# AIM-Harvard/pyradiomics

Hardware: AMD Instinct MI355X
Metric: Mvoxels/s for GLCM+GLRLM build, 512^3 vol @32 bins (higher is better)
Workload: dtype u8 levels / u32 counts / f64 out; 1 GPU; GLCM+GLRLM matrix build, 512^3 int32+uint8 volume resident in HBM, 32 grey levels, full mask, 13 angles, uniform levels; one volume per GPU (batch sharding, no collective); size=512, levels=32, dist=uniform, deferred_mode=pipeline

## Files before the change

pyradiomics_amd/csrc/kernels_sweep.h:

```cpp
#pragma once
#include "prad_runtime.h"

namespace prad {

typedef unsigned int u32;
typedef unsigned long long u64;

__global__ void __launch_bounds__(256) pack_levels_kernel(const int *__restrict__ image,
                                                          const uint8_t *__restrict__ mask, long long n, int NX,
                                                          int pitch, int padw, int Ng,
                                                          uint8_t *__restrict__ levels, int *__restrict__ flags,
                                                          int vec_ok, int shift, uint8_t *__restrict__ rowzero = nullptr) {
  const long long tid = (long long)blockIdx.x * blockDim.x + threadIdx.x;
  const long long nthreads = (long long)gridDim.x * blockDim.x;
  const bool linear = (padw == 0 && pitch == NX);
  int bad = 0;
  long long done = 0;
  if (vec_ok) {
    const long long n16 = n >> 4;
    const int upr = NX >> 4;
    const int4 *im4 = reinterpret_cast<const int4 *>(image);
    const uint4 *mk4 = reinterpret_cast<const uint4 *>(mask);
    for (long long t = tid; t < n16; t += nthreads) {
      const uint4 m = mk4[t];
// ... 66 lines not shown
  long long sM, sU;
  int LXc;
  long long chunks;
};
#define PRAD_MAX_SWEEP 16
struct SweepSet {
  int count;
  SweepDesc d[PRAD_MAX_SWEEP];
};

#define PRAD_LONG_BINS 64
struct HistLayout {
  int Ng, RS;
  bool fused;
  int glrlm0;
  int g0, RL;
  int dummy0;
  int words;
};
__host__ __device__ inline HistLayout hist_layout(bool glcm, bool glrlm, bool fused, int Ng, int RS) {
  HistLayout h;
  h.Ng = Ng;
  h.RS = RS;
  h.fused = fused;
  h.g0 = 0;
  h.RL = 0;
  if (fused) {
    h.glrlm0 = 0;
    h.g0 = (Ng + 1) * (RS + 1) * (Ng + 1);
    h.RL = PRAD_LONG_BINS;
    h.dummy0 = h.g0 + Ng * h.RL;
  } else {
    h.glrlm0 = glcm ? Ng * Ng : 0;
    h.dummy0 = h.glrlm0 + (glrlm ? RS * Ng : 0);
  }
  h.words = h.dummy0 + 64;
  return h;
}

__device__ __forceinline__ int select_i32(bool cond, int a, int b) {
  asm volatile("" : "+v"(a), "+v"(b));
  return cond ? a : b;
}

typedef __attribute__((address_space(3))) u32 lds_u32;
__device__ __forceinline__ void lds_bump(int lds_addr) {
#ifdef PRAD_DBG_NOBUMP
  asm volatile("" ::"v"(lds_addr));
  return;
#endif
  __hip_atomic_fetch_add((lds_u32 *)(size_t)(unsigned)lds_addr, 1u, __ATOMIC_RELAXED, __HIP_MEMORY_SCOPE_WORKGROUP);
}

template <bool DO_GLCM, bool DO_GLRLM, bool LONG, bool FUSED>
struct Walker {
  u32 *rl_long;
  int Ng4, Nr;
  int cG, cR;
  int rl_limit;
  int dummy;
  int prev;
  int prowG;
  int rlN;
  int nmask;

  __device__ __forceinline__ void init(u32 *lds_, const HistLayout &h, int Nr_, u32 *rl_long_, int lane) {
    const int base = (int)(unsigned)(size_t)((lds_u32 *)lds_);
    rl_long = rl_long_;
    Ng4 = 4 * h.Ng;
    Nr = Nr_;
    cG = base - 4 * (h.Ng + 1);
    cR = base + 4 * (h.glrlm0 - (h.Ng + 1));
    rl_limit = h.RS * Ng4 + cR;
    dummy = base + 4 * (h.dummy0 + lane);
  }
  __device__ __forceinline__ void begin_line() {
    prev = 0;
    prowG = cG;
    rlN = Ng4 + cR;
    nmask = 0;
  }
  __device__ __forceinline__ bool risky(int steps) const { return LONG && DO_GLRLM && rlN + steps * Ng4 > rl_limit; }
  template <bool CHECK = true>
  __device__ __forceinline__ void step(int cur) {
    const bool pnz = prev != 0, cnz = cur != 0;
    if (DO_GLCM) {
      lds_bump((pnz && cnz) ? prowG + (cur << 2) : dummy);
      prowG = __mul24(cur, Ng4) + cG;
    }
    if (DO_GLRLM) {
      const bool chg = cur != prev;
      const bool emit = chg && pnz;
      if (LONG && CHECK) {
        const bool lng = rlN > rl_limit;
        lds_bump((emit && !lng) ? rlN + (prev << 2) : dummy);
        if (emit && lng) atomicAdd(&rl_long[(size_t)(prev - 1) * Nr + ((rlN - cR) / Ng4 - 1)], 1u);
      } else {
        lds_bump(emit ? rlN + (prev << 2) : dummy);
      }
      rlN = select_i32(chg, Ng4 + cR, rlN + Ng4);
      nmask += cnz;
    }
    prev = cur;
  }
  __device__ __forceinline__ bool end_line() {
    step<true>(0);
// ... 540 lines not shown
  if ((int)blockIdx.x < nb1) {
    const long long idx = (long long)blockIdx.x * blockDim.x + threadIdx.x;
    const long long total = (long long)Ng * Ng * Na;
    if (idx >= total) return;
    const int a = (int)(idx % Na);
    const long long ij = idx / Na;
    const int i = (int)(ij / Ng), j = (int)(ij - (long long)i * Ng);
    if (i == j) return;
    glcm_out[idx] = (double)glcm_acc[(size_t)a * Ng * Ng + ij];
    return;
  }
  const int pair = ((int)blockIdx.x - nb1) * 4 + (int)(threadIdx.x >> 6), lane = threadIdx.x & 63;
  if (pair >= Ng * Na) return;
  const int i = pair % Ng, a = pair / Ng;
  u32 *row = glrlm_acc + ((size_t)a * Ng + i) * Nr;
  unsigned long long pairs = 0, longer = 0;
  int found = 0;
  for (int r = lane; r < Nr; r += 64) {
    const u32 v = row[r];
    pairs += (unsigned long long)r * v;
    if (r > 0) longer += v;
    found |= (r > 0 && v != 0);
  }
  const u32 *grow = glcm_acc + ((size_t)a * Ng + i) * Ng;
  for (int j = lane; j < Ng; j += 64) found |= (grow[j] != 0);
  for (int o = 32; o > 0; o >>= 1) pairs += __shfl_xor(pairs, o);
  if (lane == 0) glcm_out[((size_t)i * Ng + i) * Na + a] = (double)pairs;
  if (__ballot(found) != 0 && lane == 0) multi[a] = 1;
  if (restore_from >= 0 && a != restore_from) {
    const u32 *xrow = glrlm_acc + ((size_t)restore_from * Ng + i) * Nr;
    unsigned long long nvox = 0;
    for (int r = lane; r < Nr; r += 64) nvox += (unsigned long long)(r + 1) * xrow[r];
    for (int o = 32; o > 0; o >>= 1) {
      nvox += __shfl_xor(nvox, o);
      longer += __shfl_xor(longer, o);
    }
    if (lane == 0) row[0] = (u32)(nvox - (pairs + longer));
  }
}

__global__ void finalize_glrlm_kernel(const u32 *__restrict__ acc, const int *__restrict__ multi, int Ng, int Nr,
                                      int Na, double *__restrict__ out, const int *__restrict__ flags = nullptr,
                                      int *__restrict__ sticky = nullptr) {
  if (sticky && blockIdx.x == 0 && threadIdx.x == 0 && (flags[0] || flags[2])) sticky[0] = 1;
  const long long idx = (long long)blockIdx.x * blockDim.x + threadIdx.x;
  const long long total = (long long)Ng * Nr * Na;
  if (idx >= total) return;
  const int a = (int)(idx % Na);
  const long long gr = idx / Na;
  const int r = (int)(gr % Nr);
  out[idx] = (r == 0 && !multi[a]) ? 0.0 : (double)acc[(size_t)a * Ng * Nr + gr];
}

}
```

pyradiomics_amd/csrc/kernels_sweepfw.h:

```cpp
#pragma once
#include "kernels_sweep.h"

namespace prad {

enum FwPhase { FP_INIT, FP_GRAB, FP_CTRL, FP_ISSUE, FP_WAIT_ROWS, FP_WAIT_PACK, FP_GROUP, FP_PACK, FP_SLOW, FP_FLUSH, FP_DRAIN,
               FP_TOTAL, FP_REALTIME, FP_NGROUP, FP_NGROUP_PACK, FP_NSLOW, FP_COUNT };
#ifdef PRAD_FW_STAMPS
__device__ unsigned long long prad_fw_stamps[2 * 8192 * FP_COUNT];
struct FwClock {
  unsigned long long last, first, rt0;
  unsigned acc[FP_COUNT];
  __device__ __forceinline__ void start() {
#pragma unroll
    for (int i = 0; i < FP_COUNT; i++) acc[i] = 0;
    rt0 = __builtin_amdgcn_s_memrealtime();
    first = last = __builtin_readcyclecounter();
  }
  template <int PH>
  __device__ __forceinline__ void lap() {
    const unsigned long long now = __builtin_readcyclecounter();
    acc[PH] += (unsigned)(now - last);
    last = now;
  }
  template <int PH>
  __device__ __forceinline__ void count() { acc[PH]++; }
  __device__ __forceinline__ void store(int slot) {
    acc[FP_TOTAL] = (unsigned)(__builtin_readcyclecounter() - first);
    acc[FP_REALTIME] = (unsigned)(__builtin_amdgcn_s_memrealtime() - rt0);
    const unsigned w = blockIdx.x * (blockDim.x >> 6) + (threadIdx.x >> 6);
    if ((threadIdx.x & 63) == 0 && w < 8192) {
#pragma unroll
      for (int i = 0; i < FP_COUNT; i++) prad_fw_stamps[((size_t)slot * 8192 + w) * FP_COUNT + i] = acc[i];
    }
  }
};
#else
struct FwClock {
  __device__ __forceinline__ void start() {}
  template <int PH>
  __device__ __forceinline__ void lap() {}
  template <int PH>
  __device__ __forceinline__ void count() {}
  __device__ __forceinline__ void store(int) {}
};
#endif

struct FwDesc {
  int slot;
  int NM, NU;
  int du, dx;
  long long sM, sU;
  int CL, pieces;
  int chunks;
  int dom_kind;
};
struct FwSet {
  int count;
  int NX;
  int pitch;
  int nrows;
  int xcd;
  int first_block[PRAD_MAX_SWEEP + 1];
  FwDesc d[PRAD_MAX_SWEEP];
};

struct PackJob {
  const int *image;
  const uint8_t *mask;
  uint8_t *levels;
  uint8_t *levels16;
  uint8_t *rowzero;
  int *flags;
  long long n16;
  int NX, Ng;
  int every;
};

#define PRAD_FW_U 8
#ifndef PRAD_FW_MAXG
#define PRAD_FW_MAXG 4
#endif
#define PRAD_FW_WORK_STRIDE 64
#define PRAD_FW_DOMAINS 8
__host__ __device__ inline size_t fw_lds_bytes(const HistLayout &h) { return 4 * ((size_t)h.words + (size_t)(h.Ng + 1)); }


struct FwTab {
  u32 *rl_long;
  int Nr, P4, Q, lenlim, gB, RL4, RS, RL, dummy0b, alive0, deadmax;
  unsigned Qinv;
  __device__ __forceinline__ void init(const HistLayout &h, int Nr_, u32 *rl_long_) {
    rl_long = rl_long_;
    Nr = Nr_;
    Q = 4 * (h.Ng + 1);
    P4 = (h.RS + 1) * (h.Ng + 1);
    lenlim = (h.RS + 1) * Q;
// ... 671 lines not shown
          ri -= (long long)du * NU * sUr;
          zpos = 65;
          wrap = false;
          continue;
        }
        t++;
        zpos++;
        row += du;
        off += delta;
        ri += dri;
        if (du != 0 && (row < 0 || row >= NU)) wrap = true;
      }
    }
  }
};

template <bool ZA>
__device__ __forceinline__ void fw_row_word(const FwTab &T, u32 one, int &s, u32 c, u32 x) {
  int t;
#define PRAD_FW_RCOL(J)                                                                                          \
  "v_cmpx_ne_u32_sdwa vcc, %[c], %[x] src0_sel:BYTE_" #J " src1_sel:BYTE_" #J "\n\t"                             \
  "v_add_u32_sdwa %[t], %[s], %[c] dst_sel:DWORD dst_unused:UNUSED_PAD src0_sel:DWORD src1_sel:BYTE_" #J "\n\t"   \
  "v_mul_u32_u24_sdwa %[s], %[P4], %[c] dst_sel:DWORD dst_unused:UNUSED_PAD src0_sel:DWORD src1_sel:BYTE_" #J "\n\t" \
  "v_cmpx_ne_u32_sdwa vcc, %[x], %[z] src0_sel:BYTE_" #J " src1_sel:DWORD\n\t"                                  \
  "ds_add_u32 %[t], %[one]\n\t"                                                                                  \
  "s_mov_b64 exec, -1\n\t"                                                                                       \
  "v_add_u32 %[s], %[Q], %[s]\n\t"
#define PRAD_FW_RCOL_NZ(J)                                                                                       \
  "v_cmpx_ne_u32_sdwa vcc, %[c], %[x] src0_sel:BYTE_" #J " src1_sel:BYTE_" #J "\n\t"                             \
  "v_add_u32_sdwa %[t], %[s], %[c] dst_sel:DWORD dst_unused:UNUSED_PAD src0_sel:DWORD src1_sel:BYTE_" #J "\n\t"   \
  "ds_add_u32 %[t], %[one]\n\t"                                                                                  \
  "v_mul_u32_u24_sdwa %[s], %[P4], %[c] dst_sel:DWORD dst_unused:UNUSED_PAD src0_sel:DWORD src1_sel:BYTE_" #J "\n\t" \
  "s_mov_b64 exec, -1\n\t"                                                                                       \
  "v_add_u32 %[s], %[Q], %[s]\n\t"
  if (ZA) {
    u32 z = 0;
    asm volatile("" : "+v"(z));
    asm volatile(PRAD_FW_RCOL(0) PRAD_FW_RCOL(1) PRAD_FW_RCOL(2) PRAD_FW_RCOL(3)
                 : [s] "+v"(s), [t] "=&v"(t)
                 : [c] "v"(c), [x] "v"(x), [one] "v"(one), [P4] "s"(T.P4), [Q] "s"(T.Q), [z] "v"(z)
                 : "vcc", "memory");
  } else {
    asm volatile(PRAD_FW_RCOL_NZ(0) PRAD_FW_RCOL_NZ(1) PRAD_FW_RCOL_NZ(2) PRAD_FW_RCOL_NZ(3)
                 : [s] "+v"(s), [t] "=&v"(t)
                 : [c] "v"(c), [x] "v"(x), [one] "v"(one), [P4] "s"(T.P4), [Q] "s"(T.Q)
                 : "vcc", "memory");
  }
#undef PRAD_FW_RCOL
#undef PRAD_FW_RCOL_NZ
}

template <bool LONG, bool ZA>
__device__ __forceinline__ void fw_rows_role(const HistLayout &h, const FwTab &T, u32 *lds, const uint8_t *__restrict__ L,
                                             long long nrows, int NX, int pitch, int bx, int nblocks) {
  const int lane = threadIdx.x & 63, wave = threadIdx.x >> 6, wpb = blockDim.x >> 6;
  const int dummy = T.dummy0b + 4 * lane;
  u32 one = 1;
  asm volatile("" : "+v"(one));
  uint8_t *tile = reinterpret_cast<uint8_t *>(lds) + ((fw_lds_bytes(h) + 15) & ~(size_t)15) + (size_t)wave * 64 * PRAD_ROW_PITCH;
  const int RSTEP = nrows >= 4096 ? 8 : 1;
  const long long ngroups = RSTEP == 8 ? ((nrows + 511) / 512) * 8 : (nrows + 63) / 64;
  const long long nwaves = (long long)nblocks * wpb;
  const bool vec16 = (pitch & 15) == 0 && ((uintptr_t)L & 15) == 0;
  for (long long grp = (long long)bx * wpb + wave; grp < ngroups; grp += nwaves) {
    const long long r0 = RSTEP == 8 ? (grp >> 3) * 512 + (grp & 7) : grp * 64;
    int s = 0;
    u32 pw = 0;
    uint4 nx4[4];
    auto fetch = [&](int xc) __attribute__((always_inline)) {
#pragma unroll
      for (int j = 0; j < 4; j++) {
        const int rr = j * 16 + (lane >> 2);
        const int cx = xc + (lane & 3) * 16;
        uint4 q = make_uint4(0, 0, 0, 0);
        if (r0 + RSTEP * rr < nrows && cx < NX) {
          q = *reinterpret_cast<const uint4 *>(L + (r0 + RSTEP * rr) * pitch + cx);
          const int valid = NX - cx;
          if (valid < 16) {
            u32 *qw = reinterpret_cast<u32 *>(&q);
#pragma unroll
            for (int wd = 0; wd < 4; wd++) {
              const int keep = valid - 4 * wd;
              qw[wd] = keep >= 4 ? qw[wd] : (keep <= 0 ? 0u : (qw[wd] & ((1u << (8 * keep)) - 1u)));
            }
          }
        }
        nx4[j] = q;
      }
    };
    if (vec16) fetch(0);
    for (int xc = 0; xc < NX; xc += 64) {
      if (vec16) {
#pragma unroll
        for (int j = 0; j < 4; j++) *reinterpret_cast<uint4 *>(tile + (j * 16 + (lane >> 2)) * PRAD_ROW_PITCH + (lane & 3) * 16) = nx4[j];
        __builtin_amdgcn_wave_barrier();
        if (xc + 64 < NX) fetch(xc + 64);
      } else {
        const bool xin = xc + lane < NX;
#pragma unroll 8
        for (int rr = 0; rr < 64; rr++) {
          uint8_t b = 0;
          if (xin && r0 + RSTEP * rr < nrows) b = L[(r0 + RSTEP * rr) * pitch + xc + lane];
          tile[rr * PRAD_ROW_PITCH + lane] = b;
        }
      }
      __builtin_amdgcn_wave_barrier();
      const uint4 *row = reinterpret_cast<const uint4 *>(tile + lane * PRAD_ROW_PITCH);
#pragma unroll
      for (int q = 0; q < 4; q++) {
        const uint4 d = row[q];
        const u32 wds[4] = {d.x, d.y, d.z, d.w};
        const unsigned m = (pw >> 24) ? (unsigned)(s - __mul24((int)(pw >> 24), T.P4)) : 0u;
        if (LONG && __ballot(m + 16 * T.Q > (unsigned)T.lenlim) != 0) {
#pragma unroll 1
          for (int k = 0; k < 4; k++) {
            const u32 c = wds[k], x = __builtin_amdgcn_alignbyte(c, pw, 3);
            const unsigned m4 = (pw >> 24) ? (unsigned)(s - __mul24((int)(pw >> 24), T.P4)) : 0u;
            if (__ballot(m4 + 4 * T.Q > (unsigned)T.lenlim) != 0) {
#pragma unroll
              for (int b = 0; b < 4; b++) fw_checked<LONG>(T, dummy, s, (int)((x >> (8 * b)) & 0xffu), (int)((c >> (8 * b)) & 0xffu), false);
            } else {
              fw_row_word<ZA>(T, one, s, c, x);
            }
            pw = c;
          }
        } else {
#pragma unroll
          for (int k = 0; k < 4; k++) {
            fw_row_word<ZA>(T, one, s, wds[k], __builtin_amdgcn_alignbyte(wds[k], pw, 3));
            pw = wds[k];
          }
        }
      }
      __builtin_amdgcn_wave_barrier();
    }
    fw_checked<LONG>(T, dummy, s, (int)(pw >> 24), 0, false);
  }
}

template <bool LONG>
__global__ void __launch_bounds__(1024) sweep_fw_rows_kernel(const uint8_t *__restrict__ L, long long nrows, int NX, int pitch,
                                                            int slot, int Ng, int Nr, int RS, u32 *__restrict__ glcm_acc,
                                                            u32 *__restrict__ glrlm_acc, int *__restrict__ flags) {
  extern __shared__ u32 lds[];
  if (flags[0]) return;
  const HistLayout h = hist_layout(true, true, true, Ng, RS);
  if ((unsigned)(size_t)((lds_u32 *)lds) != 0u) {
    if (threadIdx.x == 0) atomicExch(flags + 2, 1);
    return;
  }
  for (int i = threadIdx.x; i < h.words + Ng + 1; i += blockDim.x) lds[i] = 0;
  __syncthreads();
  FwTab T;
  T.init(h, Nr, glrlm_acc + (size_t)slot * Ng * Nr);
  if (flags[3] != 0) fw_rows_role<LONG, true>(h, T, lds, L, nrows, NX, pitch, (int)blockIdx.x, (int)gridDim.x);
  else fw_rows_role<LONG, false>(h, T, lds, L, nrows, NX, pitch, (int)blockIdx.x, (int)gridDim.x);
  flush_block_hist<true, true, true>(lds + Ng + 1, h, Nr, slot, glcm_acc, glrlm_acc);
}

template <bool LONG, int K, bool HASPAD, bool PACK>
__global__ void __launch_bounds__(1024) sweep_fw_kernel(FwSet set, PackJob pj, const uint8_t *__restrict__ L,
                                                        const uint8_t *__restrict__ rowzero, int Ng, int Nr, int RS,
                                                        u32 *__restrict__ glcm_acc, u32 *__restrict__ glrlm_acc,
                                                        int *__restrict__ work, int *__restrict__ flags) {
  extern __shared__ u32 lds[];
  int role = 0;
  while (role + 1 < set.count && (int)blockIdx.x >= set.first_block[role + 1]) role++;
  const int bx = (int)blockIdx.x - set.first_block[role], nblocks = set.first_block[role + 1] - set.first_block[role];
  const int wpb = (int)(blockDim.x >> 6);
  const long long pw = __builtin_amdgcn_readfirstlane((int)(blockIdx.x * wpb + (threadIdx.x >> 6)));
  PackWave pk(pj, pw, (long long)gridDim.x * wpb);
  FwClock clk;
  clk.start();
#ifdef PRAD_FW_SETPRIO
  __builtin_amdgcn_s_setprio(PRAD_FW_SETPRIO);
#endif
  if (flags[0] == 0) {
    const bool anyzero = flags[3] != 0;
    const HistLayout h = hist_layout(true, true, true, Ng, RS);
    if ((unsigned)(size_t)((lds_u32 *)lds) != 0u) {
      if (threadIdx.x == 0) atomicExch(flags + 2, 1);
    } else {
      for (int i = threadIdx.x; i < h.words + Ng + 1; i += blockDim.x) lds[i] = 0;
      __syncthreads();
      clk.lap<FP_INIT>();
      const FwDesc &D = set.d[role];
      FwTab T;
      T.init(h, Nr, glrlm_acc + (size_t)D.slot * Ng * Nr);
      int *wk = work + PRAD_FW_WORK_STRIDE * PRAD_FW_DOMAINS * role;
      if (D.dx == 0) {
        FwWave<LONG, K, 0, HASPAD, PACK> w(T, set.NX);
        w.run(D, set.NX, set.pitch, set.nrows, L, rowzero, anyzero, wk, bx, nblocks, pk, pj, set.xcd != 0, clk);
      } else if (D.dx > 0) {
        FwWave<LONG, K, 1, HASPAD, PACK> w(T, set.NX);
        w.run(D, set.NX, set.pitch, set.nrows, L, rowzero, anyzero, wk, bx, nblocks, pk, pj, set.xcd != 0, clk);
      } else {
        FwWave<LONG, K, -1, HASPAD, PACK> w(T, set.NX);
        w.run(D, set.NX, set.pitch, set.nrows, L, rowzero, anyzero, wk, bx, nblocks, pk, pj, set.xcd != 0, clk);
      }
      clk.lap<FP_CTRL>();
      flush_block_hist<true, true, true>(lds + Ng + 1, h, Nr, D.slot, glcm_acc, glrlm_acc);
      clk.lap<FP_FLUSH>();
    }
  }
  if (PACK) pk.drain(pj);
  clk.lap<FP_DRAIN>();
  clk.store(PACK ? 1 : 0);
}

}
// ... 1 lines not shown
```

pyradiomics_amd/csrc/kernels_sweepfw2.h:

```cpp
#pragma once
#include "kernels_sweepfw.h"

namespace prad {

struct Fw2Tab {
  u32 *rl_long;
  int Nr, Ng, RS2, C;
  int S, S4, K1, lenlim;
  __device__ __forceinline__ void init(int Ng_, int RS2_, int C_, int Nr_, u32 *rl_long_) {
    rl_long = rl_long_;
    Nr = Nr_;
    Ng = Ng_;
    RS2 = RS2_;
    C = C_;
    S4 = Ng_ + 1 + C_ * RS2_;
    S = 4 * S4;
    K1 = 4 * Ng_;
    lenlim = 4 * RS2_;
  }
};
__host__ __device__ inline size_t fw2_table_words(int Ng, int RS2, int C) { return (size_t)(Ng + 1) * (size_t)(Ng + 1 + C * RS2); }

__device__ __noinline__ void fw2_long_event(const Fw2Tab &T, int lv, int idx) {
  const unsigned key = ((unsigned)lv << 20) | (unsigned)idx;
// ... 627 lines not shown
    const int bx = (int)blockIdx.x - set.first_block[role], nblocks = set.first_block[role + 1] - set.first_block[role];
    const int words = (int)fw2_table_words(Ng, RS2, C);
    for (int i = threadIdx.x; i < words; i += blockDim.x) lds[i] = 0;
    __syncthreads();
    const FwDesc &D = set.d[role];
    Fw2Tab T;
    T.init(Ng, RS2, C, Nr, glrlm_acc + (size_t)D.slot * Ng * Nr);
    int *wk = work + PRAD_FW_WORK_STRIDE * PRAD_FW_DOMAINS * role;
    if (D.dx == 0) {
      Fw2Wave<LONG, K, 0, HASPAD, SKIP1, PACK> w(T, set.NX);
      w.run(D, set.NX, set.pitch, set.nrows, L, wk, bx, nblocks, set.xcd != 0, pk, pj);
    } else if (D.dx > 0) {
      Fw2Wave<LONG, K, 1, HASPAD, SKIP1, PACK> w(T, set.NX);
      w.run(D, set.NX, set.pitch, set.nrows, L, wk, bx, nblocks, set.xcd != 0, pk, pj);
    } else {
      Fw2Wave<LONG, K, -1, HASPAD, SKIP1, PACK> w(T, set.NX);
      w.run(D, set.NX, set.pitch, set.nrows, L, wk, bx, nblocks, set.xcd != 0, pk, pj);
    }
    fw2_flush(lds, T, D.slot, glcm_acc, glrlm_acc);
  }
  if (PACK) pk.drain(pj);
}

#define PRAD_ROW16_EL 32
#define PRAD_ROW16_PITCH 80
__device__ __forceinline__ void fw2_row_word(const Fw2Tab &T, int k1, u32 one, int &p, int &q, u32 c, u32 x) {
  int t;
#define PRAD_FW2_RCOL(J)                                                                                                 \
  "v_cmpx_ne_u32_sdwa vcc, %[c], %[x] src0_sel:WORD_" #J " src1_sel:WORD_" #J "\n\t"                                     \
  "v_add_u32_sdwa %[t], %[p], %[c] dst_sel:DWORD dst_unused:UNUSED_PAD src0_sel:DWORD src1_sel:WORD_" #J "\n\t"            \
  "ds_add_u32 %[t], %[one]\n\t"                                                                                          \
  "ds_add_u32 %[q], %[one]\n\t"                                                                                          \
  "v_mul_u32_u24_sdwa %[p], %[S4], %[c] dst_sel:DWORD dst_unused:UNUSED_PAD src0_sel:DWORD src1_sel:WORD_" #J "\n\t"      \
  "v_add_u32 %[q], %[K1], %[p]\n\t"                                                                                      \
  "s_mov_b64 exec, -1\n\t"                                                                                               \
  "v_add_u32 %[q], 4, %[q]\n\t"
  asm volatile(PRAD_FW2_RCOL(0) PRAD_FW2_RCOL(1)
               : [p] "+v"(p), [q] "+v"(q), [t] "=&v"(t)
               : [c] "v"(c), [x] "v"(x), [one] "v"(one), [S4] "s"(T.S4), [K1] "v"(k1)
               : "vcc", "memory");
#undef PRAD_FW2_RCOL
}

template <bool LONG>
__global__ void __launch_bounds__(1024) sweep_fw2_rows_kernel(const uint8_t *__restrict__ L16, long long nrows, int NX, int pitch16,
                                                             int slot, int Ng, int Nr, int RS2, int C, u32 *__restrict__ glcm_acc,
                                                             u32 *__restrict__ glrlm_acc, int *__restrict__ flags) {
  extern __shared__ u32 lds[];
  if (flags[0]) return;
  if ((unsigned)(size_t)((lds_u32 *)lds) != 0u) {
    if (threadIdx.x == 0) atomicExch(flags + 2, 1);
    return;
  }
  const int words = (int)fw2_table_words(Ng, RS2, C);
  for (int i = threadIdx.x; i < words; i += blockDim.x) lds[i] = 0;
  __syncthreads();
  Fw2Tab T;
  T.init(Ng, RS2, C, Nr, glrlm_acc + (size_t)slot * Ng * Nr);
  const int lane = threadIdx.x & 63, wave = threadIdx.x >> 6, wpb = blockDim.x >> 6;
  const int dummy = 4 * lane;
  u32 one = 1;
  int k1v = T.K1 + (lane % T.C) * T.lenlim;
  asm volatile("" : "+v"(one), "+v"(k1v));
  uint8_t *tile = reinterpret_cast<uint8_t *>(lds) + ((4 * (size_t)words + 15) & ~(size_t)15) + (size_t)wave * 64 * PRAD_ROW16_PITCH;
  const int RSTEP = nrows >= 4096 ? 8 : 1;
  const long long ngroups = RSTEP == 8 ? ((nrows + 511) / 512) * 8 : (nrows + 63) / 64;
  const long long nwaves = (long long)gridDim.x * wpb;
  for (long long grp = (long long)blockIdx.x * wpb + wave; grp < ngroups; grp += nwaves) {
    const long long r0 = RSTEP == 8 ? (grp >> 3) * 512 + (grp & 7) : grp * 64;
    int p = 0, q = k1v;
    u32 pw = 0;
    uint4 nx4[4];
    auto fetch = [&](int xc) __attribute__((always_inline)) {
#pragma unroll
      for (int j = 0; j < 4; j++) {
        const int rr = j * 16 + (lane >> 2);
        const int cx = xc + (lane & 3) * 8;
        uint4 v = make_uint4(0, 0, 0, 0);
        if (r0 + (long long)RSTEP * rr < nrows && cx < NX) {
          v = *reinterpret_cast<const uint4 *>(L16 + (r0 + (long long)RSTEP * rr) * pitch16 + 2 * cx);
          const int valid = NX - cx;
          if (valid < 8) {
            u32 *vw = reinterpret_cast<u32 *>(&v);
#pragma unroll
            for (int wd = 0; wd < 4; wd++) {
              const int keep = valid - 2 * wd;
              vw[wd] = keep >= 2 ? vw[wd] : (keep <= 0 ? 0u : (vw[wd] & 0xffffu));
            }
          }
        }
        nx4[j] = v;
      }
    };
    fetch(0);
    for (int xc = 0; xc < NX; xc += PRAD_ROW16_EL) {
#pragma unroll
      for (int j = 0; j < 4; j++) *reinterpret_cast<uint4 *>(tile + (j * 16 + (lane >> 2)) * PRAD_ROW16_PITCH + (lane & 3) * 16) = nx4[j];
      __builtin_amdgcn_wave_barrier();
      if (xc + PRAD_ROW16_EL < NX) fetch(xc + PRAD_ROW16_EL);
      const uint4 *row = reinterpret_cast<const uint4 *>(tile + lane * PRAD_ROW16_PITCH);
#pragma unroll 2
      for (int qd = 0; qd < PRAD_ROW16_EL / 8; qd++) {
        const uint4 d = row[qd];
        const u32 wds[4] = {d.x, d.y, d.z, d.w};
        q = select_i32(p < T.S, k1v, q);
        if (LONG && __ballot((unsigned)(q - p - k1v) + 32u > (unsigned)T.lenlim) != 0) {
#pragma unroll
          for (int k = 0; k < 4; k++) {
            const u32 c = wds[k], x = __builtin_amdgcn_alignbyte(c, pw, 2);
#pragma unroll
            for (int b = 0; b < 2; b++)
              fw2_checked<LONG, false>(T, k1v, dummy, p, q, (int)((x >> (16 * b)) & 0xffffu), (int)((c >> (16 * b)) & 0xffffu), false);
            pw = c;
          }
        } else {
#pragma unroll
          for (int k = 0; k < 4; k++) {
            fw2_row_word(T, k1v, one, p, q, wds[k], __builtin_amdgcn_alignbyte(wds[k], pw, 2));
            pw = wds[k];
          }
        }
      }
      __builtin_amdgcn_wave_barrier();
    }
    fw2_checked<LONG, false>(T, k1v, dummy, p, q, (int)(pw >> 16), 0, false);
  }
  fw2_flush(lds, T, slot, glcm_acc, glrlm_acc);
}

__global__ void __launch_bounds__(256) pack_levels16_kernel(const int *__restrict__ image, const uint8_t *__restrict__ mask,
                                                            long long n, int NX, int pitch16, int pitch8, int Ng,
                                                            uint8_t *__restrict__ L16, uint8_t *__restrict__ L8,
                                                            int *__restrict__ flags) {
  const long long tid = (long long)blockIdx.x * blockDim.x + threadIdx.x;
  const long long nthreads = (long long)gridDim.x * blockDim.x;
  int bad = 0;
  if ((NX & 3) == 0) {
    const long long n4 = n >> 2;
    const int upr = NX >> 2;
    for (long long t = tid; t < n4; t += nthreads) {
      const int4 q = reinterpret_cast<const int4 *>(image)[t];
      const u32 m = reinterpret_cast<const u32 *>(mask)[t];
      const int lv[4] = {q.x, q.y, q.z, q.w};
      u32 e[4];
#pragma unroll
      for (int b = 0; b < 4; b++) {
        const bool in = (m >> (8 * b)) & 0xffu;
        const bool regular = in && lv[b] >= 1 && lv[b] <= Ng;
        bad |= in && !regular;
        e[b] = regular ? (u32)lv[b] : 0u;
      }
      const long long row = t / upr;
      const int x = (int)(t - row * upr) << 2;
      *reinterpret_cast<uint2 *>(L16 + row * pitch16 + 2 * x) =
          make_uint2((e[0] << PRAD_FUSED_SHIFT) | (e[1] << (16 + PRAD_FUSED_SHIFT)), (e[2] << PRAD_FUSED_SHIFT) | (e[3] << (16 + PRAD_FUSED_SHIFT)));
      if (L8) *reinterpret_cast<u32 *>(L8 + row * pitch8 + x) = e[0] | (e[1] << 8) | (e[2] << 16) | (e[3] << 24);
    }
  } else {
    for (long long i = tid; i < n; i += nthreads) {
      const bool in = mask[i] != 0;
      const int l = image[i];
      const bool regular = in && l >= 1 && l <= Ng;
      bad |= in && !regular;
      const long long row = i / NX;
      const int x = (int)(i - row * NX);
      *reinterpret_cast<unsigned short *>(L16 + row * pitch16 + 2 * x) = (unsigned short)(regular ? (l << PRAD_FUSED_SHIFT) : 0);
      if (L8) L8[row * pitch8 + x] = (uint8_t)(regular ? l : 0);
    }
  }
  if (bad) flags[0] = 1;
}

}
```

pyradiomics_amd/csrc/prad_api.hip:

```cpp
#include "prad_runtime.h"
#include "kernels_generic.h"
#include "kernels_pairs.h"
#include "kernels_sweep.h"
#include "kernels_sweepfw.h"
#include "kernels_sweepfw2.h"
#include "kernels_neigh.h"
#include "kernels_glszm.h"
#include "kernels_voxel.h"
#include "kernels_voxslide.h"
#include "kernels_mcc.h"
#include "kernels_voxtex.h"
#include "kernels_binning.h"

#include <algorithm>
#include <atomic>
#include <chrono>
#include <cmath>
#include <condition_variable>
#include <cstdlib>
#include <deque>
#include <limits>
#include <mutex>
#include <thread>

// ... 820 lines not shown
        PRAD_TRY((launch_rows<G, R, false, F>(k, p, v.levels, v.Ng, v.Nr, v.glcm_acc, v.glrlm_acc, v.multi)));
      }
    }
    return PRAD_OK;
  }
  Timed t(*k.c, "sweep", k.s);
  if (p.lines.count > 0) {
    if (R && p.LONG) PRAD_TRY((launch_lines<G, R, true, F>(k, p, v.levels, v.Ng, v.Nr, v.glcm_acc, v.glrlm_acc, v.multi)));
    else PRAD_TRY((launch_lines<G, R, false, F>(k, p, v.levels, v.Ng, v.Nr, v.glcm_acc, v.glrlm_acc, v.multi)));
  }
  if (p.row_slot >= 0) {
    if (R && p.LONGr) PRAD_TRY((launch_rows<G, R, true, F>(k, p, v.levels, v.Ng, v.Nr, v.glcm_acc, v.glrlm_acc, v.multi)));
    else PRAD_TRY((launch_rows<G, R, false, F>(k, p, v.levels, v.Ng, v.Nr, v.glcm_acc, v.glrlm_acc, v.multi)));
  }
  return PRAD_OK;
}

int vol_sweep(Call &k, const VolState &v, const PackJob &pj) {
  if (pj.n16 > 0 && !pipeline_volume(v.p, v.glcm != nullptr, v.glrlm != nullptr))
    return fail(PRAD_E_ARG, "internal: a pack job needs a fixed-window host launch");
  if (pj.n16 > 0 && (pj.levels16 != nullptr) != v.p.fw2)
    return fail(PRAD_E_ARG, "internal: the pack job's layout is not the host launch's");
  if (v.glcm && v.glrlm && v.p.fused) return launch_sweeps<true, true, true>(k, v, pj);
  if (v.glcm && v.glrlm) return launch_sweeps<true, true, false>(k, v, pj);
  if (v.glcm) return launch_sweeps<true, false, false>(k, v, pj);
  return launch_sweeps<false, true, false>(k, v, pj);
}

__global__ void latch_flags_kernel(const int *__restrict__ flags, int *__restrict__ sticky) {
  if (flags[0] || flags[2]) sticky[0] = 1;
}

__global__ void latch_any_flag_kernel(const int *__restrict__ flags, int *__restrict__ sticky) {
  if (flags[0] || flags[1] || flags[2]) sticky[0] = 1;
}
int latch_neigh(Context &c, Call &k) {
  int *sticky = nullptr;
  PRAD_TRY(c.get<int>("deferred_sticky", 16, &sticky));
  hipLaunchKernelGGL(latch_any_flag_kernel, dim3(1), dim3(1), 0, k.s, (const int *)k.flags_d, sticky);
  return check_launch("latch_any_flag_kernel");
}

int vol_finalize(Call &k, const VolState &v, int *sticky) {
  Context &c = *k.c;
  const SweepPlan &p = v.p;
  const int Ng = v.Ng, Nr = v.Nr, Na = v.Na;
  double *glcm = v.glcm, *glrlm = v.glrlm;
  bool latched = false;
  {
    Timed t(c, "finalize", k.s);
    const bool runs_diag = p.fused || p.fw2;
    if (p.fw2 && p.skip1 && p.lines.count > 0 && !(glcm && glrlm && p.row_slot >= 0))
      return fail(PRAD_E_UNSUPPORTED, "sweep plan derives runs of length 1 but the call cannot restore them");
    if (glcm && glrlm && runs_diag) {
      const int nb1 = (int)blocks_for((long long)Ng * Ng * Na), nb2 = (Ng * Na + 3) / 4;
      hipLaunchKernelGGL(finalize_glcm_diag_kernel, dim3(nb1 + nb2), dim3(256), 0, k.s, v.glcm_acc, v.glrlm_acc, Ng, Nr, Na, nb1,
                         glcm, v.multi, (p.fw2 && p.skip1 && p.lines.count > 0) ? p.row_slot : -1);
      PRAD_TRY(check_launch("finalize_glcm_diag_kernel"));
    } else if (glcm) {
      hipLaunchKernelGGL(finalize_glcm_kernel, dim3(blocks_for((long long)Ng * Ng * Na)), dim3(256), 0, k.s,
                         v.glcm_acc, v.glrlm_acc, Ng, Nr, Na, p.fused ? 1 : 0, glcm);
      PRAD_TRY(check_launch("finalize_glcm_kernel"));
    }
    if (glrlm && runs_diag) {
      if (!glcm) {
        hipLaunchKernelGGL(glcm_diag_resolve_kernel, dim3(Ng, Na), dim3(64), 0, k.s, v.glcm_acc, v.glrlm_acc, Ng, Nr, Na,
                           glcm, v.multi);
        PRAD_TRY(check_launch("glcm_diag_resolve_kernel"));
      }
      if (v.levels)
        hipLaunchKernelGGL(multi_check_kernel<uint8_t>, dim3(128, Na), dim3(256), 0, k.s, p.aset, (const uint8_t *)v.levels, p.Nz, p.Ny,
                           p.Nx, p.pitch, v.multi);
      else
        hipLaunchKernelGGL(multi_check_kernel<unsigned short>, dim3(128, Na), dim3(256), 0, k.s, p.aset,
                           reinterpret_cast<const unsigned short *>(v.levels16), p.Nz, p.Ny, p.Nx, p.pitch16 / 2, v.multi);
      PRAD_TRY(check_launch("multi_check_kernel"));
    }
    if (glrlm) {
      hipLaunchKernelGGL(finalize_glrlm_kernel, dim3(blocks_for((long long)Ng * Nr * Na)), dim3(256), 0, k.s,
                         v.glrlm_acc, v.multi, Ng, Nr, Na, glrlm, (const int *)v.flags_d, sticky);
      PRAD_TRY(check_launch("finalize_glrlm_kernel"));
      latched = sticky != nullptr;
    }
  }
  if (sticky && !latched) {
    hipLaunchKernelGGL(latch_flags_kernel, dim3(1), dim3(1), 0, k.s, v.flags_d, sticky);
    PRAD_TRY(check_launch("latch_flags_kernel"));
  }
  return PRAD_OK;
}

int sweep_glcm_glrlm(Call &k, const SweepPlan &p, int Ng, int Nr, double *glcm, double *glrlm, bool *used) {
  Context &c = *k.c;
  VolState v;
  PRAD_TRY(vol_prepare(k, p, Ng, Nr, glcm, glrlm, v));
  PRAD_TRY(vol_pack_standalone(k, v));
  PackJob pj;
  memset(&pj, 0, sizeof(pj));
  PRAD_TRY(vol_sweep(k, v, pj));
  int *sticky = nullptr;
  if (c.deferred) PRAD_TRY(c.get<int>("deferred_sticky", 16, &sticky));
  PRAD_TRY(vol_finalize(k, v, sticky));
  if (c.deferred) {
    *used = true;
    return PRAD_OK;
  }
// ... 712 lines not shown
}

#include "prad_voxel.h"

}

namespace prad {
int zone_features_launch(Context &c, hipStream_t s, const double *P, int Ni, int Njcap, long long stride_i,
                         const double *jvals_d, const int *nj_dev, double *out_d, int *empty_d);
}
#define ZM_FEATURES 16
namespace {
template <typename T>
int launch_digitize(const T *image, const uint8_t *mask, long long n, const double *e_d, int nedges, int32_t *levels,
                    int *top, unsigned long long *counts_d, hipStream_t s) {
  static const int cap = getenv("PRAD_BIN_BLOCKS") ? atoi(getenv("PRAD_BIN_BLOCKS")) : 1024;
  const unsigned gx = (unsigned)std::max<long long>(1, std::min<long long>((n + 255) / 256, cap));
  const size_t edge_b = sizeof(double) * (size_t)nedges, cnt_b = 4 * sizeof(unsigned) * ((size_t)nedges + 1);
  const bool lds_edges = edge_b <= 60 * 1024;
  const size_t cnt3_b = 256 * sizeof(unsigned) * ((size_t)nedges + 1);
  const int counts = !counts_d ? 0 : (nedges <= 48 ? 3 : ((lds_edges && edge_b + cnt_b <= 64 * 1024) ? 1 : 2));
#define PRAD_DIG(LE, CN)                                                                                              \
  hipLaunchKernelGGL((digitize_kernel<T, LE, CN>), dim3(gx), dim3(256),                                               \
                     (LE ? edge_b : 0) + (CN == 1 ? cnt_b : (CN == 3 ? cnt3_b : 0)), s, image, mask, n, e_d, nedges, levels, top, counts_d)
  if (lds_edges) {
    if (counts == 0) PRAD_DIG(true, 0);
    else if (counts == 1) PRAD_DIG(true, 1);
    else if (counts == 3) PRAD_DIG(true, 3);
    else PRAD_DIG(true, 2);
  } else {
    if (counts == 0) PRAD_DIG(false, 0);
    else PRAD_DIG(false, 2);
  }
#undef PRAD_DIG
  return check_launch("digitize_kernel");
}
}

extern "C" {

const char *prad_version(void) { return kVersion; }
const char *prad_last_error(void) { return err_state().msg; }
const char *prad_last_path(void) { return ctx().last_path; }
const char *prad_last_variant(void) { return ctx().last_variant; }
#ifdef PRAD_FW_STAMPS
int prad_debug_fw_stamps(unsigned long long *out, int slot, int nwaves) {
  if (!out || nwaves < 1 || nwaves > 8192 || slot < 0 || slot > 1) return PRAD_E_ARG;
  PRAD_HIP(hipDeviceSynchronize());
  PRAD_HIP(hipMemcpyFromSymbol(out, HIP_SYMBOL(prad::prad_fw_stamps), sizeof(unsigned long long) * prad::FP_COUNT * (size_t)nwaves,
                               sizeof(unsigned long long) * prad::FP_COUNT * 8192 * (size_t)slot));
  return PRAD_OK;
}
#endif

int prad_device_count(void) {
  int n = 0;
  if (hipGetDeviceCount(&n) != hipSuccess) return 0;
  return n;
}

int prad_set_device(int device) {
  int n = prad_device_count();
  if (device < 0 || device >= n) return fail(PRAD_E_ARG, "device %d not in [0,%d)", device, n);
  Context &c = ctx();
  if (c.device != device) {
    if (pipe_state().pending.valid && c.device_set && hipSetDevice(c.device) == hipSuccess) {
      (void)pipeline_flush(c);
      if (pipe_state().s) (void)hipStreamSynchronize(pipe_state().s);
      (void)fin_join(nullptr, true);
    }
    pipe_state().pending.valid = false;
    pipe_state().s = nullptr;
    pipe_state().ev = nullptr;
    pipe_state().fin = nullptr;
    for (int l = 0; l < 4; l++) pipe_state().fin_used[l] = false;
    c.own_stream = nullptr;
    for (int l = 0; l < PRAD_MAX_LANES; l++) {
      if (c.lane_stream[l]) (void)hipStreamSynchronize(c.lane_stream[l]);
      c.lane_stream[l] = nullptr;
      c.lane_in[l] = nullptr;
    }
    c.event_pool.clear();
    c.events_used = 0;
  }
  c.device = device;
  c.device_set = true;
  PRAD_HIP(hipSetDevice(device));
  return PRAD_OK;
}
int prad_get_device(void) { return ctx().device; }

long long prad_workspace_bytes(void) {
  long long total = 0;
  for (const auto &kv : ctx().bufs) total += (long long)kv.second.cap;
  return total;
}
namespace {
void release_image_queues();
}
int prad_release_workspace(void) {
  Context &c = ctx();
  if (pipe_state().pending.valid) {
    (void)pipeline_flush(c);
    if (pipe_state().s) (void)hipStreamSynchronize(pipe_state().s);
    (void)fin_join(nullptr, true);
    pipe_state().pending.valid = false;
// ... 771 lines not shown
```

Before: 287,900 Mvoxels/s.

## Fuse finalize kernels into one launch and batch row tile LDS reads

```diff
diff --git a/pyradiomics_amd/csrc/kernels_sweep.h b/pyradiomics_amd/csrc/kernels_sweep.h
--- a/pyradiomics_amd/csrc/kernels_sweep.h
+++ b/pyradiomics_amd/csrc/kernels_sweep.h
@@ -142,6 +142,23 @@
   __hip_atomic_fetch_add((lds_u32 *)(size_t)(unsigned)lds_addr, 1u, __ATOMIC_RELAXED, __HIP_MEMORY_SCOPE_WORKGROUP);
 }
 
+__device__ __forceinline__ void lds_read_row64(unsigned addr, uint4 (&d)[4]) {
+  typedef u32 v4u __attribute__((ext_vector_type(4)));
+  v4u a, b, c, e;
+  asm volatile("ds_read_b128 %0, %4\n\t"
+               "ds_read_b128 %1, %4 offset:16\n\t"
+               "ds_read_b128 %2, %4 offset:32\n\t"
+               "ds_read_b128 %3, %4 offset:48\n\t"
+               "s_waitcnt lgkmcnt(0)"
+               : "=&v"(a), "=&v"(b), "=&v"(c), "=&v"(e)
+               : "v"(addr)
+               : "memory");
+  d[0] = make_uint4(a.x, a.y, a.z, a.w);
+  d[1] = make_uint4(b.x, b.y, b.z, b.w);
+  d[2] = make_uint4(c.x, c.y, c.z, c.w);
+  d[3] = make_uint4(e.x, e.y, e.z, e.w);
+}
+
 template <bool DO_GLCM, bool DO_GLRLM, bool LONG, bool FUSED>
 struct Walker {
   u32 *rl_long;
@@ -788,4 +805,100 @@
   out[idx] = (r == 0 && !multi[a]) ? 0.0 : (double)acc[(size_t)a * Ng * Nr + gr];
 }
 
-}
+template <typename T>
+__global__ void __launch_bounds__(1024) finalize_both_kernel(AngleSet A, const T *__restrict__ L, int Nz, int Ny, int Nx, int pitch,
+                                                             const u32 *__restrict__ glcm_acc, const u32 *__restrict__ glrlm_acc,
+                                                             const int *__restrict__ multi, int Ng, int Nr, int Na, int b1, int b2,
+                                                             int restore_from, double *__restrict__ glcm_out,
+                                                             double *__restrict__ glrlm_out, const int *__restrict__ flags,
+                                                             int *__restrict__ sticky) {
+  const int bid = (int)blockIdx.x, tid = (int)threadIdx.x, nt = (int)blockDim.x;
+  if (bid >= b2) {
+    const long long idx = (long long)(bid - b2) * nt + tid;
+    if (idx >= (long long)Ng * Nr * Na) return;
+    const int a = (int)(idx % Na);
+    const long long gr = idx / Na;
+    if ((int)(gr % Nr) == 0) return;
+    glrlm_out[idx] = (double)glrlm_acc[(size_t)a * Ng * Nr + gr];
+    return;
+  }
+  if (bid >= b1) {
+    const int pair = (bid - b1) * (nt >> 6) + (tid >> 6), lane = tid & 63;
+    if (pair >= Ng * Na) return;
+    const int i = pair % Ng, a = pair / Ng;
+    const u32 *row = glrlm_acc + ((size_t)a * Ng + i) * Nr;
+    unsigned long long pairs = 0;
+    for (int r = lane; r < Nr; r += 64) pairs += (unsigned long long)r * row[r];
+    for (int o = 32; o > 0; o >>= 1) pairs += __shfl_xor(pairs, o);
+    if (lane == 0) glcm_out[((size_t)i * Ng + i) * Na + a] = (double)pairs;
+    return;
+  }
+  if (bid >= Na) {
+    const long long idx = (long long)(bid - Na) * nt + tid;
+    if (idx >= (long long)Ng * Ng * Na) return;
+    const int a = (int)(idx % Na);
+    const long long ij = idx / Na;
+    const int i = (int)(ij / Ng), j = (int)(ij - (long long)i * Ng);
+    if (i == j) return;
+    glcm_out[idx] = (double)glcm_acc[(size_t)a * Ng * Ng + ij];
+    return;
+  }
+  const int a = bid;
+  const bool skipped = flags && (flags[0] || flags[2]);
+  if (sticky && a == 0 && tid == 0 && skipped) sticky[0] = 1;
+  int found = multi[a] != 0;
+  {
+    const u32 *racc = glrlm_acc + (size_t)a * Ng * Nr;
+    for (int w = tid; w < Ng * Nr; w += nt) found |= (w % Nr != 0 && racc[w] != 0);
+    const u32 *gacc = glcm_acc + (size_t)a * Ng * Ng;
+    for (int w = tid; w < Ng * Ng; w += nt) found |= gacc[w] != 0;
+  }
+  found = __syncthreads_or(found);
+  if (!found && !skipped) {
+    const int dz = A.off[a][0], dy = A.off[a][1], dx = A.off[a][2];
+    const long long nfz = dz ? (long long)Ny * Nx : 0, nfy = dy ? (long long)Nz * Nx : 0, nfx = dx ? (long long)Nz * Ny : 0;
+    for (long long s0 = 0; s0 < nfz + nfy + nfx && !found; s0 += nt) {
+      const long long s = s0 + tid;
+      int cnt = 0;
+      if (s < nfz + nfy + nfx) {
+        int z, y, x;
+        if (s < nfz) {
+          z = dz > 0 ? 0 : Nz - 1; y = (int)(s / Nx); x = (int)(s - (long long)y * Nx);
+        } else if (s < nfz + nfy) {
+          const long long t = s - nfz;
+          y = dy > 0 ? 0 : Ny - 1; z = (int)(t / Nx); x = (int)(t - (long long)z * Nx);
+        } else {
+          const long long t = s - nfz - nfy;
+          x = dx > 0 ? 0 : Nx - 1; z = (int)(t / Ny); y = (int)(t - (long long)z * Ny);
+        }
+        while (cnt < 2 && (unsigned)z < (unsigned)Nz && (unsigned)y < (unsigned)Ny && (unsigned)x < (unsigned)Nx) {
+          cnt += L[((long long)z * Ny + y) * pitch + x] != 0;
+          z += dz; y += dy; x += dx;
+        }
+      }
+      found = __syncthreads_or(cnt > 1);
+    }
+  }
+  if (!found) {
+    for (int i = tid; i < Ng; i += nt) glrlm_out[((size_t)i * Nr) * Na + a] = 0.0;
+  } else if (restore_from < 0 || a == restore_from) {
+    for (int i = tid; i < Ng; i += nt) glrlm_out[((size_t)i * Nr) * Na + a] = (double)glrlm_acc[((size_t)a * Ng + i) * Nr];
+  } else {
+    const int lane = tid & 63;
+    for (int i = tid >> 6; i < Ng; i += nt >> 6) {
+      const u32 *row = glrlm_acc + ((size_t)a * Ng + i) * Nr, *xrow = glrlm_acc + ((size_t)restore_from * Ng + i) * Nr;
+      unsigned long long nvox = 0, longer = 0;
+      for (int r = lane; r < Nr; r += 64) {
+        nvox += (unsigned long long)(r + 1) * xrow[r];
+        if (r > 0) longer += (unsigned long long)(r + 1) * row[r];
+      }
+      for (int o = 32; o > 0; o >>= 1) {
+        nvox += __shfl_xor(nvox, o);
+        longer += __shfl_xor(longer, o);
+      }
+      if (lane == 0) glrlm_out[((size_t)i * Nr) * Na + a] = (double)(u32)(nvox - longer);
+    }
+  }
+}
+
+}
diff --git a/pyradiomics_amd/csrc/kernels_sweepfw.h b/pyradiomics_amd/csrc/kernels_sweepfw.h
--- a/pyradiomics_amd/csrc/kernels_sweepfw.h
+++ b/pyradiomics_amd/csrc/kernels_sweepfw.h
@@ -42,6 +42,53 @@
   template <int PH>
   __device__ __forceinline__ void count() {}
   __device__ __forceinline__ void store(int) {}
+};
+#endif
+
+enum RowsPhase { RP_INIT, RP_STAGE, RP_WALK, RP_SYNC, RP_FLUSH, RP_TOTAL, RP_REALTIME, RP_NTILES, RP_COUNT };
+#ifdef PRAD_FW_ROWS_STAMPS
+__device__ unsigned long long prad_fw_rows_stamps[8192 * RP_COUNT];
+struct RowsClock {
+  unsigned long long last, first, rt0;
+  unsigned acc[RP_COUNT];
+  __device__ __forceinline__ void start() {
+#pragma unroll
+    for (int i = 0; i < RP_COUNT; i++) acc[i] = 0;
+    rt0 = __builtin_amdgcn_s_memrealtime();
+    first = last = __builtin_readcyclecounter();
+  }
+  template <int PH>
+  __device__ __forceinline__ void lap() {
+    asm volatile("s_waitcnt lgkmcnt(0)" ::: "memory");
+    const unsigned long long now = __builtin_readcyclecounter();
+    acc[PH] += (unsigned)(now - last);
+    last = now;
+  }
+  template <int PH>
+  __device__ __forceinline__ void count() { acc[PH]++; }
+  __device__ __forceinline__ void sync() {
+    __syncthreads();
+    lap<RP_SYNC>();
+  }
+  __device__ __forceinline__ void store() {
+    acc[RP_TOTAL] = (unsigned)(__builtin_readcyclecounter() - first);
+    acc[RP_REALTIME] = (unsigned)(__builtin_amdgcn_s_memrealtime() - rt0);
+    const unsigned w = blockIdx.x * (blockDim.x >> 6) + (threadIdx.x >> 6);
+    if ((threadIdx.x & 63) == 0 && w < 8192) {
+#pragma unroll
+      for (int i = 0; i < RP_COUNT; i++) prad_fw_rows_stamps[(size_t)w * RP_COUNT + i] = acc[i];
+    }
+  }
+};
+#else
+struct RowsClock {
+  __device__ __forceinline__ void start() {}
+  template <int PH>
+  __device__ __forceinline__ void lap() {}
+  template <int PH>
+  __device__ __forceinline__ void count() {}
+  __device__ __forceinline__ void sync() {}
+  __device__ __forceinline__ void store() {}
 };
 #endif
 
@@ -819,12 +866,13 @@
 
 template <bool LONG, bool ZA>
 __device__ __forceinline__ void fw_rows_role(const HistLayout &h, const FwTab &T, u32 *lds, const uint8_t *__restrict__ L,
-                                             long long nrows, int NX, int pitch, int bx, int nblocks) {
+                                             long long nrows, int NX, int pitch, int bx, int nblocks, RowsClock &clk) {
   const int lane = threadIdx.x & 63, wave = threadIdx.x >> 6, wpb = blockDim.x >> 6;
   const int dummy = T.dummy0b + 4 * lane;
   u32 one = 1;
   asm volatile("" : "+v"(one));
   uint8_t *tile = reinterpret_cast<uint8_t *>(lds) + ((fw_lds_bytes(h) + 15) & ~(size_t)15) + (size_t)wave * 64 * PRAD_ROW_PITCH;
+  const unsigned tile_lds = (unsigned)(tile - reinterpret_cast<uint8_t *>(lds));
   const int RSTEP = nrows >= 4096 ? 8 : 1;
   const long long ngroups = RSTEP == 8 ? ((nrows + 511) / 512) * 8 : (nrows + 63) / 64;
   const long long nwaves = (long long)nblocks * wpb;
@@ -872,10 +920,13 @@
         }
       }
       __builtin_amdgcn_wave_barrier();
-      const uint4 *row = reinterpret_cast<const uint4 *>(tile + lane * PRAD_ROW_PITCH);
+      uint4 rowq[4];
+      lds_read_row64(tile_lds + (unsigned)lane * PRAD_ROW_PITCH, rowq);
+      clk.template lap<RP_STAGE>();
+      clk.template count<RP_NTILES>();
 #pragma unroll
       for (int q = 0; q < 4; q++) {
-        const uint4 d = row[q];
+        const uint4 d = rowq[q];
         const u32 wds[4] = {d.x, d.y, d.z, d.w};
         const unsigned m = (pw >> 24) ? (unsigned)(s - __mul24((int)(pw >> 24), T.P4)) : 0u;
         if (LONG && __ballot(m + 16 * T.Q > (unsigned)T.lenlim) != 0) {
@@ -900,6 +951,7 @@
         }
       }
       __builtin_amdgcn_wave_barrier();
+      clk.template lap<RP_WALK>();
     }
     fw_checked<LONG>(T, dummy, s, (int)(pw >> 24), 0, false);
   }
@@ -916,13 +968,20 @@
     if (threadIdx.x == 0) atomicExch(flags + 2, 1);
     return;
   }
+  RowsClock clk;
+  clk.start();
   for (int i = threadIdx.x; i < h.words + Ng + 1; i += blockDim.x) lds[i] = 0;
   __syncthreads();
+  clk.lap<RP_INIT>();
   FwTab T;
   T.init(h, Nr, glrlm_acc + (size_t)slot * Ng * Nr);
-  if (flags[3] != 0) fw_rows_role<LONG, true>(h, T, lds, L, nrows, NX, pitch, (int)blockIdx.x, (int)gridDim.x);
-  else fw_rows_role<LONG, false>(h, T, lds, L, nrows, NX, pitch, (int)blockIdx.x, (int)gridDim.x);
+  if (flags[3] != 0) fw_rows_role<LONG, true>(h, T, lds, L, nrows, NX, pitch, (int)blockIdx.x, (int)gridDim.x, clk);
+  else fw_rows_role<LONG, false>(h, T, lds, L, nrows, NX, pitch, (int)blockIdx.x, (int)gridDim.x, clk);
+  clk.lap<RP_WALK>();
+  clk.sync();
   flush_block_hist<true, true, true>(lds + Ng + 1, h, Nr, slot, glcm_acc, glrlm_acc);
+  clk.lap<RP_FLUSH>();
+  clk.store();
 }
 
 template <bool LONG, int K, bool HASPAD, bool PACK>
diff --git a/pyradiomics_amd/csrc/kernels_sweepfw2.h b/pyradiomics_amd/csrc/kernels_sweepfw2.h
--- a/pyradiomics_amd/csrc/kernels_sweepfw2.h
+++ b/pyradiomics_amd/csrc/kernels_sweepfw2.h
@@ -703,9 +703,12 @@
     if (threadIdx.x == 0) atomicExch(flags + 2, 1);
     return;
   }
+  RowsClock clk;
+  clk.start();
   const int words = (int)fw2_table_words(Ng, RS2, C);
   for (int i = threadIdx.x; i < words; i += blockDim.x) lds[i] = 0;
   __syncthreads();
+  clk.lap<RP_INIT>();
   Fw2Tab T;
   T.init(Ng, RS2, C, Nr, glrlm_acc + (size_t)slot * Ng * Nr);
   const int lane = threadIdx.x & 63, wave = threadIdx.x >> 6, wpb = blockDim.x >> 6;
@@ -714,6 +717,7 @@
   int k1v = T.K1 + (lane % T.C) * T.lenlim;
   asm volatile("" : "+v"(one), "+v"(k1v));
   uint8_t *tile = reinterpret_cast<uint8_t *>(lds) + ((4 * (size_t)words + 15) & ~(size_t)15) + (size_t)wave * 64 * PRAD_ROW16_PITCH;
+  const unsigned tile_lds = (unsigned)(tile - reinterpret_cast<uint8_t *>(lds));
   const int RSTEP = nrows >= 4096 ? 8 : 1;
   const long long ngroups = RSTEP == 8 ? ((nrows + 511) / 512) * 8 : (nrows + 63) / 64;
   const long long nwaves = (long long)gridDim.x * wpb;
@@ -749,10 +753,14 @@
       for (int j = 0; j < 4; j++) *reinterpret_cast<uint4 *>(tile + (j * 16 + (lane >> 2)) * PRAD_ROW16_PITCH + (lane & 3) * 16) = nx4[j];
       __builtin_amdgcn_wave_barrier();
       if (xc + PRAD_ROW16_EL < NX) fetch(xc + PRAD_ROW16_EL);
-      const uint4 *row = reinterpret_cast<const uint4 *>(tile + lane * PRAD_ROW16_PITCH);
-#pragma unroll 2
+      static_assert(PRAD_ROW16_EL == 32, "lds_read_row64 reads 64 bytes per row");
+      uint4 rowq[4];
+      lds_read_row64(tile_lds + (unsigned)lane * PRAD_ROW16_PITCH, rowq);
+      clk.lap<RP_STAGE>();
+      clk.count<RP_NTILES>();
+#pragma unroll
       for (int qd = 0; qd < PRAD_ROW16_EL / 8; qd++) {
-        const uint4 d = row[qd];
+        const uint4 d = rowq[qd];
         const u32 wds[4] = {d.x, d.y, d.z, d.w};
         q = select_i32(p < T.S, k1v, q);
         if (LONG && __ballot((unsigned)(q - p - k1v) + 32u > (unsigned)T.lenlim) != 0) {
@@ -773,10 +781,15 @@
         }
       }
       __builtin_amdgcn_wave_barrier();
+      clk.lap<RP_WALK>();
     }
     fw2_checked<LONG, false>(T, k1v, dummy, p, q, (int)(pw >> 16), 0, false);
   }
+  clk.lap<RP_WALK>();
+  clk.sync();
   fw2_flush(lds, T, slot, glcm_acc, glrlm_acc);
+  clk.lap<RP_FLUSH>();
+  clk.store();
 }
 
 __global__ void __launch_bounds__(256) pack_levels16_kernel(const int *__restrict__ image, const uint8_t *__restrict__ mask,
diff --git a/pyradiomics_amd/csrc/prad_api.hip b/pyradiomics_amd/csrc/prad_api.hip
--- a/pyradiomics_amd/csrc/prad_api.hip
+++ b/pyradiomics_amd/csrc/prad_api.hip
@@ -896,6 +896,23 @@
     const bool runs_diag = p.fused || p.fw2;
     if (p.fw2 && p.skip1 && p.lines.count > 0 && !(glcm && glrlm && p.row_slot >= 0))
       return fail(PRAD_E_UNSUPPORTED, "sweep plan derives runs of length 1 but the call cannot restore them");
+    if (glcm && glrlm && runs_diag && (v.levels || v.levels16)) {
+      const int T = 1024;
+      const long long ng = ((long long)Ng * Ng * Na + T - 1) / T, nd = ((long long)Ng * Na + T / 64 - 1) / (T / 64),
+                      nr = ((long long)Ng * Nr * Na + T - 1) / T;
+      const int b1 = Na + (int)ng, b2 = b1 + (int)nd;
+      const int restore = (p.fw2 && p.skip1 && p.lines.count > 0) ? p.row_slot : -1;
+      if (v.levels)
+        hipLaunchKernelGGL(finalize_both_kernel<uint8_t>, dim3((unsigned)(b2 + nr)), dim3(T), 0, k.s, p.aset, (const uint8_t *)v.levels,
+                           p.Nz, p.Ny, p.Nx, p.pitch, v.glcm_acc, v.glrlm_acc, v.multi, Ng, Nr, Na, b1, b2, restore, glcm, glrlm,
+                           (const int *)v.flags_d, sticky);
+      else
+        hipLaunchKernelGGL(finalize_both_kernel<unsigned short>, dim3((unsigned)(b2 + nr)), dim3(T), 0, k.s, p.aset,
+                           reinterpret_cast<const unsigned short *>(v.levels16), p.Nz, p.Ny, p.Nx, p.pitch16 / 2, v.glcm_acc,
+                           v.glrlm_acc, v.multi, Ng, Nr, Na, b1, b2, restore, glcm, glrlm, (const int *)v.flags_d, sticky);
+      PRAD_TRY(check_launch("finalize_both_kernel"));
+      return PRAD_OK;
+    }
     if (glcm && glrlm && runs_diag) {
       const int nb1 = (int)blocks_for((long long)Ng * Ng * Na), nb2 = (Ng * Na + 3) / 4;
       hipLaunchKernelGGL(finalize_glcm_diag_kernel, dim3(nb1 + nb2), dim3(256), 0, k.s, v.glcm_acc, v.glrlm_acc, Ng, Nr, Na, nb1,
@@ -1714,6 +1731,14 @@
   return PRAD_OK;
 }
 #endif
+#ifdef PRAD_FW_ROWS_STAMPS
+int prad_debug_fw_rows_stamps(unsigned long long *out, int nwaves) {
+  if (!out || nwaves < 1 || nwaves > 8192) return PRAD_E_ARG;
+  PRAD_HIP(hipDeviceSynchronize());
+  PRAD_HIP(hipMemcpyFromSymbol(out, HIP_SYMBOL(prad::prad_fw_rows_stamps), sizeof(unsigned long long) * prad::RP_COUNT * (size_t)nwaves, 0));
+  return PRAD_OK;
+}
+#endif
 
 int prad_device_count(void) {
   int n = 0;
```

Result: no change. 288,900 Mvoxels/s, median of 6 (+0.3%).
